# dkogan/mrcal

Measured on AMD Instinct MI355X. Metric: LM (dog-leg) iterations/sec, 8-cam x 1000-frame OPENCV8 calibration, higher is better.
Workload: dtype f64; 1 GPU; 8 cameras x 1000 frames x 10x10 corners, LENSMODEL_OPENCV8, all variables optimized, warp + regularization; Nstate=6140, Nmeasurements=1600080, Nnz_J=37200080, parallelism=single GPU

## Files before the change

mrcal_amd/csrc/assembly.hip:

```cpp
#include "solver_device.hpp"
#include "assembly_splined.hpp"
#include "solver_kernel_decls.hpp"

namespace mrcal_amd {




__device__ __forceinline__
void assemble_frame_block(const DeviceProblem& P, const NormalDims& nd, const OpDev& O, const AssemblyPlan& plan,
                          const double* __restrict__ gram, int f, int o0, int o1 ,
                          int mode, bool do_factor, double lambda,
                          const FactorBuffers& F, double* __restrict__ lds_f)
{
    double* __restrict__ Btf  = lds_f;
    double* __restrict__ Df   = lds_f + 6*nd.Nc;
    double* __restrict__ gf   = Df + 36;
    double* __restrict__ Ls   = gf + 6;
    double* __restrict__ rinv = Ls + 36;
    const int t = threadIdx.x;
#ifdef ASM_TS
    long long ats[16]; int nats = 0;
#define ATS() do { if(t == 0 && nats < 16) ats[nats++] = clock64(); } while(0)
#else
#define ATS()
#endif
    ATS();
    const int e0 = 6*f;
    double* __restrict__ Bt = O.Bt;
    double* __restrict__ D  = O.D;
    double* __restrict__ g  = O.g;

    if(mode == 1)
    {
        for(int i = t; i < 6*nd.Nc + 42; i += blockDim.x) lds_f[i] = 0.0;
        __syncthreads();
        const int npos = gram_stride(P.Ndist);
        for(int ob = o0; ob < o1; ob += 8)
        {
            int col_i[8], col_e[8];
            int obs[8];
#pragma unroll
            for(int u = 0; u < 8; u++)
            {
                const int i = (ob + u < o1) ? ob + u : o0;
                obs[u] = plan.frame_obs ? plan.frame_obs[i] : i;
            }
#pragma unroll
            for(int u = 0; u < 8; u++) { col_i[u] = plan.obs_cols[2*obs[u]]; col_e[u] = plan.obs_cols[2*obs[u]+1]; }
            for(int base = 0; base < npos; base += 2*blockDim.x)
            {
                const int pos0 = base + t;
                double vv[2][8];
                int    rec[2];
#pragma unroll
                for(int w = 0; w < 2; w++)
                {
                    const int pos = pos0 + w*blockDim.x;
                    const int pc  = (pos < npos) ? pos : t;
                    rec[w] = (pos < npos) ? plan.frame_pos[pc] : FRAMEPOS_NONE;
#pragma unroll
                    for(int u = 0; u < 8; u++) vv[w][u] = 0.0;
                    if((rec[w] & 7) != FRAMEPOS_NONE)
                    {
#pragma unroll
                        for(int u = 0; u < 8; u++) vv[w][u] = gram[(size_t)obs[u]*npos + pc];
                    }
                }
#pragma unroll
                for(int w = 0; w < 2; w++)
                {
                    const int kind = rec[w] & 7, a = (rec[w] >> 3) & 7, k = rec[w] >> 6;
                    if(kind == FRAMEPOS_NONE) continue;
                    if(kind == FRAMEPOS_BT_INTRINSICS || kind == FRAMEPOS_BT_EXTRINSICS)
                    {
                        double* __restrict__ row = Btf + a*nd.Nc + k;
#pragma unroll
                        for(int u = 0; u < 8; u++)
                        {
                            const int c = (kind == FRAMEPOS_BT_INTRINSICS) ? col_i[u] : col_e[u];
                            if(ob + u < o1 && c >= 0) row[c] += vv[w][u];
                        }
                    }
                    else
                    {
                        double* __restrict__ dst = (kind == FRAMEPOS_GF)      ? gf + a :
                                                   (kind == FRAMEPOS_BT_WARP) ? Btf + a*nd.Nc + k : Df + a*6 + k;
                        double acc = *dst;
#pragma unroll
                        for(int u = 0; u < 8; u++) if(ob + u < o1) acc += vv[w][u];
                        *dst = acc;
                        if(kind == FRAMEPOS_D_MIRROR) Df[k*6 + a] = acc;
                    }
                }
                ATS();
            }
        }
        __syncthreads();
        ATS();
        for(int i = t; i < 6*nd.Nc; i += blockDim.x) Bt[(size_t)e0*nd.Nc + i] = Btf[i];
        if(t < 36)      D[(size_t)f*36 + t]     = Df[t];
        else if(t < 42) g[nd.E_state0 + e0 + (t-36)] = gf[t-36];
    }
    else
    {
        for(int i = t; i < 6*nd.Nc; i += blockDim.x) Btf[i] = Bt[(size_t)e0*nd.Nc + i];
        if(t < 36)      Df[t]    = D[(size_t)f*36 + t];
        else if(t < 42) gf[t-36] = g[nd.E_state0 + e0 + (t-36)];
        __syncthreads();
    }
    if(!do_factor) return;

    if(t == 0)
    {
        double M[6][6];
#pragma unroll
        for(int i=0;i<6;i++)
#pragma unroll
            for(int j=0;j<6;j++) M[i][j] = Df[i*6+j] + ((i == j) ? lambda : 0.0);
        bool ok = true;
#pragma unroll
        for(int j=0;j<6;j++)
        {
            double d = M[j][j];
#pragma unroll
            for(int k=0;k<j;k++) d -= M[j][k]*M[j][k];
            if(!(d > 0.0)) { ok = false; d = 1.0; }
            d = sqrt(d);
            const double rd = 1.0/d;
            M[j][j] = d;
            rinv[j] = rd;
#pragma unroll
            for(int i=j+1;i<6;i++)
            {
                double v = M[i][j];
#pragma unroll
                for(int k=0;k<j;k++) v -= M[i][k]*M[j][k];
                M[i][j] = v*rd;
            }
        }
#pragma unroll
        for(int i=0;i<6;i++)
#pragma unroll
            for(int j=0;j<6;j++) Ls[i*6+j] = (j <= i) ? M[i][j] : 0.0;
        if(!ok) atomicExch(F.status, 1);
    }
    ATS();
    __syncthreads();
    ATS();
    if(t < 36) F.LD[(size_t)f*36 + t] = Ls[t];
    double Lr[6][6], ri[6];
#pragma unroll
    for(int i=0;i<6;i++)
    {
        ri[i] = rinv[i];
#pragma unroll
        for(int k=0;k<i;k++) Lr[i][k] = Ls[i*6+k];
    }
    for(int c = t; c <= nd.Nc; c += blockDim.x)
    {
        double w[6];
#pragma unroll
        for(int i=0;i<6;i++)
        {
            double v = (c < nd.Nc) ? Btf[i*nd.Nc + c] : gf[i];
#pragma unroll
            for(int k=0;k<i;k++) v -= Lr[i][k]*w[k];
            w[i] = v*ri[i];
        }
        if(c < nd.Nc) { for(int i=0;i<6;i++) F.Wt[(size_t)(e0+i)*nd.Nc + c] = w[i]; }
        else          { for(int i=0;i<6;i++) F.y[e0+i] = w[i]; }
    }
    ATS();
#ifdef ASM_TS
    if(t == 0 && (f == 0 || f == 300 || f == 999))
        printf("asm ts f=%d n=%d (zero | loads + adds | sync | bt-write+factor | sync | fsub): %lld %lld %lld %lld %lld %lld\n", f, nats,
               ats[1]-ats[0], ats[2]-ats[1], ats[3]-ats[2], ats[4]-ats[3], ats[5]-ats[4], ats[6]-ats[5]);
#endif
}

__device__ __forceinline__
void reduce_pair_chunk(const DeviceProblem& P, const AssemblyPlan& plan,
                       const double* __restrict__ gram, int ichunk, int islice )
{
    const int c0 = plan.chunk_begin[ichunk], c1 = plan.chunk_begin[ichunk+1];
    const int npos = gram_stride(P.Ndist);
    const PairOp* __restrict__ ops = plan.pair_table + (size_t)plan.chunk_pair[ichunk]*npos;
    double* __restrict__ out = plan.chunk_part + (size_t)ichunk*npos;
    const int nobs = c1 - c0;
#ifdef ASM_TS
    const long long cts0 = clock64();
#endif
    const int  pos  = islice*blockDim.x + threadIdx.x;
    const int  kind = (pos < npos) ? (ops[pos].op & 0xff) : PAIROP_NONE;
    const bool live = (kind == PAIROP_A || kind == PAIROP_G || kind == PAIROP_NORM);
    double acc = 0.0;
    for(int u0 = 0; u0 < nobs; u0 += 16)
    {
        double vv[16];
        unsigned ob[16];
#pragma unroll
        for(int u = 0; u < 16; u++)
        {
            const int k = (u0 + u < nobs) ? c0 + u0 + u : c0;
            ob[u] = (unsigned)plan.pair_obs[k]*(unsigned)npos;
        }
#pragma unroll
        for(int u = 0; u < 16; u++) vv[u] = 0.0;
        if(live)
        {
// ... 772 lines not shown
```

mrcal_amd/csrc/cholesky_lds.hip:

```cpp
#include "solver_device.hpp"
#include "chol_diag16.hpp"
#include "solver_kernel_decls.hpp"
#include "step_device.hpp"

namespace mrcal_amd {


template<int FINISH>
__device__ __forceinline__
void schur_cholesky_solve_body(int n, const int* __restrict__ skip, int keep_factor,
                               double* __restrict__ S, double* __restrict__ r,
                               int* __restrict__ status, const Step2Dev& sd, const double* __restrict__ Spk = NULL)
{
    if(skip != NULL && *skip) return;
    if constexpr(FINISH == 1) { if(!step2_finish(sd, status)) return; }
    extern __shared__ __attribute__((aligned(16))) double Mp[];
    const int t    = threadIdx.x;
    const int nt   = blockDim.x;
    const int lane = t & 63, wave = t >> 6;
    const int wave_u = __builtin_amdgcn_readfirstlane(wave);
    const int npanels = (n + CHOL_PB - 1)/CHOL_PB;
    const int r16 = lane & 15, kq = lane >> 4;

    auto rowptr = [&](int i) -> double* { return Mp + ((i*(i+1)) >> 1); };
    double* __restrict__ Xs   = Mp + chol_tri_doubles(n);
    double* __restrict__ cbuf = Xs + npanels*CHOL_PB*CHOL_XLD;

    __shared__ int notpd;
    if(t == 0) notpd = 0;
#ifdef CHOL_TS
    long long cts[64]; int ncts = 0;
#define CTS() do { if(t == 0 && ncts < 64) cts[ncts++] = clock64(); } while(0)
#else
#define CTS()
#endif
    CTS();

    if(Spk != NULL)
    {
        const int ntri = ((n*(n + 1)) >> 1) + n;
        const int n16 = min(n, CHOL_PB), nfirst = (n16*(n16 + 1)) >> 1;
        if(wave_u == 0)
        {
            double v[3];
#pragma unroll
            for(int u = 0; u < 3; u++) { const int idx = lane + 64*u; v[u] = Spk[idx < nfirst ? idx : 0]; }
#pragma unroll
            for(int u = 0; u < 3; u++) { const int idx = lane + 64*u; if(idx < nfirst) Mp[idx] = v[u]; }
        }
        else
        {
            constexpr int UP = 16;
            const int nt1 = nt - 64;
            for(int i0 = nfirst + (t - 64); i0 < ntri; i0 += UP*nt1)
            {
                double v[UP];
#pragma unroll
                for(int u = 0; u < UP; u++) { const int idx = i0 + u*nt1; v[u] = Spk[idx < ntri ? idx : 0]; }
#pragma unroll
                for(int u = 0; u < UP; u++) { const int idx = i0 + u*nt1; if(idx < ntri) Mp[idx] = v[u]; }
            }
        }
    }
    else
    {
        double v[13][4];
#pragma unroll
        for(int a = 0; a < 13; a++)
#pragma unroll
            for(int b = 0; b < 4; b++)
                if(b <= a/4)
                {
                    const int  i = wave_u + 16*a, j = lane + 64*b;
                    const bool ok = (i < n && j <= i);
                    v[a][b] = S[ok ? (size_t)i*n + j : 0];
                }
#pragma unroll
        for(int a = 0; a < 13; a++)
#pragma unroll
            for(int b = 0; b < 4; b++)
                if(b <= a/4)
                {
                    const int i = wave_u + 16*a, j = lane + 64*b;
                    if(i < n && j <= i) rowptr(i)[j] = v[a][b];
                }
    }
    if(Spk == NULL)
    {
        for(int j = t; j < n; j += nt) rowptr(n)[j] = r[j];
        __syncthreads();
    }

    auto factor_diag = [&](int p) __attribute__((always_inline))
    {
        const int j0 = p*CHOL_PB;
        const int jb = min(CHOL_PB, n - j0);
        const bool mine = lane < 16 && r16 < jb;
        double* __restrict__ rowL = rowptr(j0 + (mine ? r16 : 0)) + j0;
        double* __restrict__ sink = cbuf + 128 + lane;
        const bool bad = chol_factor_diag16(lane, jb, rowL, Xs + p*CHOL_PB*CHOL_XLD, cbuf,
                                            [&](int c) -> double* { return (mine && c <= r16) ? rowL + c : sink; });
        if(bad && lane == 0) notpd = 1;
    };

    CTS();
    for(int p = -1; p < npanels; p++)
    {
        const int j0 = (p < 0) ? 0 : p*CHOL_PB;
        const int jb = min(CHOL_PB, n - j0);
        const int m0 = j0 + jb;

        if(p >= 0)
        {
            const double* __restrict__ X = Xs + p*CHOL_PB*CHOL_XLD;
            const int ntile_b = (n + 1 - m0 + 15) >> 4;
            for(int ti = wave_u; ti < ntile_b; ti += 16)
            {
                const int  ia = m0 + 16*ti + r16;
                const bool va = ia <= n;
                const double* __restrict__ pa = rowptr(va ? ia : n) + j0;
                chol_double4_t acc = {0.0, 0.0, 0.0, 0.0};
#pragma unroll
                for(int s4 = 0; s4 < 4; s4++)
                {
                    const int  k  = 4*s4 + kq;
                    const bool vk = k < jb;
                    const double al = pa[vk ? k : 0];
                    const double av = (va && vk) ? al : 0.0;
                    const double bv = X[k*CHOL_XLD + r16];
                    acc = __builtin_amdgcn_mfma_f64_16x16x4f64(av, bv, acc, 0, 0, 0);
                }
#pragma unroll
                for(int v = 0; v < 4; v++)
                {
                    const int ri = m0 + 16*ti + kq + 4*v;
                    if(ri <= n && r16 < jb) rowptr(ri)[j0 + r16] = acc[v];
                }
            }
        }
        if(p >= 0) __syncthreads();
        CTS();

        {
            const int nrows = n + 1 - m0, ncols = n - m0;
            const int ntr = (p < 0) ? 0 : (nrows + 15) >> 4, ntc = (ncols + 15) >> 4;
            int ntiles = 0;
            for(int ta = 0; ta < ntr; ta++) ntiles += min(ta + 1, ntc);
            for(int tix = wave_u; tix < ntiles; tix += (wave_u == 0 ? ntiles : 15))
            {
                int ta = 0, tb = tix;
                for(;;) { const int ntb = min(ta + 1, ntc); if(tb < ntb) break; tb -= ntb; ta++; }
                {
                    const int  ia = 16*ta + r16, ib = 16*tb + r16;
                    const bool va = ia < nrows, vb = ib < ncols;
                    const double* __restrict__ pa = rowptr(m0 + (va ? ia : 0)) + j0;
                    const double* __restrict__ pb = rowptr(m0 + (vb ? ib : 0)) + j0;
                    chol_double4_t acc;
                    double* cp[4]; bool cv[4];
#pragma unroll
                    for(int v = 0; v < 4; v++)
                    {
                        const int ri = 16*ta + kq + 4*v, cj = 16*tb + r16;
                        cv[v] = (ri < nrows) && (cj < ncols) && (cj <= ri);
                        cp[v] = rowptr(m0 + (cv[v] ? ri : 0)) + m0 + (cv[v] ? cj : 0);
                        const double cval = *cp[v];
                        acc[v] = cv[v] ? cval : 0.0;
                    }
#pragma unroll
                    for(int s4 = 0; s4 < 4; s4++)
                    {
                        const int  k  = 4*s4 + kq;
                        const bool vk = k < jb;
                        const double al = pa[k], bl = pb[k];
                        const double av = (va && vk) ? -al : 0.0;
                        const double bv = (vb && vk) ?  bl : 0.0;
                        acc = __builtin_amdgcn_mfma_f64_16x16x4f64(av, bv, acc, 0, 0, 0);
                    }
#pragma unroll
                    for(int v = 0; v < 4; v++) if(cv[v]) *cp[v] = acc[v];
                }
            }
            if(wave == 0 && p + 1 < npanels)
            {
                __builtin_amdgcn_s_setprio(3);
                factor_diag(p + 1);
                __builtin_amdgcn_s_setprio(0);
            }
        }
        __syncthreads();
        CTS();
    }
    if(t == 0 && notpd) atomicExch(status, 1);


    double* __restrict__ z = rowptr(n);
    auto back_diag = [&](int p) __attribute__((always_inline))
    {
        const int j0 = p*CHOL_PB;
        const int jb = min(CHOL_PB, n - j0);
        const double* __restrict__ X = Xs + p*CHOL_PB*CHOL_XLD + ((lane < CHOL_PB) ? lane : 0)*CHOL_XLD;
        double xv[CHOL_PB], wv[CHOL_PB];
#pragma unroll
        for(int k = 0; k < CHOL_PB; k++) { xv[k] = X[k]; wv[k] = z[j0 + ((k < jb) ? k : 0)]; }
        double acc0 = 0.0, acc1 = 0.0;
#pragma unroll
        for(int k = 0; k < CHOL_PB; k += 2)
        {
            acc0 += (k   < jb && k   >= lane) ? xv[k]  *wv[k]   : 0.0;
            acc1 += (k+1 < jb && k+1 >= lane) ? xv[k+1]*wv[k+1] : 0.0;
        }
        if(lane < jb) z[j0 + lane] = acc0 + acc1;
    };
    auto back_update = [&](int i, int j0, int jb) __attribute__((always_inline))
    {
        if(jb == CHOL_PB)
        {
            const double* __restrict__ zp = z + j0;
            double lv[CHOL_PB], zv[CHOL_PB];
#pragma unroll
            for(int c = 0; c < CHOL_PB; c++) { lv[c] = rowptr(j0+c)[i]; zv[c] = zp[c]; }
            double acc0 = 0.0, acc1 = 0.0;
#pragma unroll
            for(int c = 0; c < CHOL_PB; c += 2) { acc0 += lv[c]*zv[c]; acc1 += lv[c+1]*zv[c+1]; }
            z[i] -= acc0 + acc1;
        }
        else
        {
            double acc = 0.0;
            for(int c = 0; c < jb; c++) acc += rowptr(j0+c)[i]*z[j0+c];
            z[i] -= acc;
        }
    };
    CTS();
    if(wave == 0 && npanels > 0) back_diag(npanels-1);
    __syncthreads();
    CTS();
    auto back_chain = [&](int p, double& dcur) __attribute__((always_inline))
    {
        const int j0 = p*CHOL_PB, jm = j0 - CHOL_PB, l16 = (lane < CHOL_PB) ? lane : 0;
        const int i = jm + l16;
        const double* __restrict__ X = Xs + (p - 1)*CHOL_PB*CHOL_XLD + l16*CHOL_XLD;
        double lv[CHOL_PB], xv[CHOL_PB];
#pragma unroll
        for(int c = 0; c < CHOL_PB; c++) { lv[c] = rowptr(j0+c)[i]; xv[c] = X[c]; }
        const double zi = z[i];
        double acc0 = 0.0, acc1 = 0.0;
#pragma unroll
        for(int c = 0; c < CHOL_PB; c += 2) { acc0 += lv[c]*readlane_f64(dcur, c); acc1 += lv[c+1]*readlane_f64(dcur, c+1); }
        const double w = zi - (acc0 + acc1);
        double b0 = 0.0, b1 = 0.0;
#pragma unroll
        for(int k = 0; k < CHOL_PB; k += 2)
        {
            const double w0 = readlane_f64(w, k), w1 = readlane_f64(w, k+1);
            b0 += (k   >= lane) ? xv[k]  *w0 : 0.0;
            b1 += (k+1 >= lane) ? xv[k+1]*w1 : 0.0;
        }
        dcur = b0 + b1;
        if(lane < CHOL_PB) z[jm + lane] = dcur;
    };
    double dcur = 0.0;
    bool have_dcur = false;
    for(int p = npanels-1; p >= 1; p--)
    {
        const int j0 = p*CHOL_PB;
        const int jb = min(CHOL_PB, n - j0);
        if(wave == 0)
        {
            if(have_dcur && jb == CHOL_PB) back_chain(p, dcur);
            else
            {
                if(lane < CHOL_PB) back_update(j0 - CHOL_PB + lane, j0, jb);
                back_diag(p - 1);
                dcur = z[j0 - CHOL_PB + ((lane < CHOL_PB) ? lane : 0)];
                have_dcur = true;
            }
        }
        else
            for(int i = t - 64; i < j0 - CHOL_PB; i += nt - 64) back_update(i, j0, jb);
        __syncthreads();
        CTS();
    }
    for(int i = t; i < n; i += nt) r[i] = -z[i];
    if(keep_factor)
        for(int idx = t; idx < n*n; idx += nt)
        {
            const int i = idx / n, j = idx - i*n;
            if(j <= i) S[(size_t)i*n + j] = rowptr(i)[j];
        }
    CTS();
    if constexpr(FINISH != 0) { if(t == 0) step2_chol_done(sd, notpd != 0); }
#ifdef CHOL_TS
    if(t == 0) { printf("chol ts (load | diag0 | b,c per panel ... | backward | store):"); for(int i=1;i<ncts;i++) printf(" %lld", cts[i]-cts[i-1]); printf("\n"); }
#endif
}

template<int FINISH>
__global__ __launch_bounds__(1024)
void schur_cholesky_solve_kernel(int n, const int* __restrict__ skip, int keep_factor,
                                 double* __restrict__ S, double* __restrict__ r,
                                 int* __restrict__ status, Step2Dev sd)
{
    schur_cholesky_solve_body<FINISH>(n, skip, keep_factor, S, r, status, sd);
}

__global__ __launch_bounds__(1024)
void step2_chol_quadform_kernel(int n, int* __restrict__ status, Step2Dev sd, NormalDims nd,
                                double* __restrict__ S, double* __restrict__ r, double* __restrict__ qf_part, int nqf,
                                const double* __restrict__ Spk)
{
    if(blockIdx.x == 0)
    {
// ... 106 lines not shown
```

mrcal_amd/csrc/problem.cpp:

```cpp
#include <hip/hip_runtime.h>
#include <stdlib.h>
#include <string.h>
#include <vector>
#include <map>
#include <algorithm>
#include "layout.hpp"
#include "host_state.hpp"
#include "problem.hpp"
#include "kernels.hpp"
#include "lens_dispatch.hpp"
#include "problem_object.hpp"
#include "host_copy.hpp"
#include <thread>
#include <unordered_map>
#include <mutex>
#include <condition_variable>
#include <deque>
#include <chrono>
#include <unistd.h>

using namespace mrcal_amd;

mrcal_amd_problem::~mrcal_amd_problem()
{
// ... 397 lines not shown
                default: break;
                }
            };
            bool consistent = true;
            for(size_t ip = 0; ip < pair_rep.size(); ip++)
                for(int pos = 0; pos < npos; pos++)
                {
                    int kind, a, k, base;
                    classify(ptab[ip*npos + pos], &kind, &a, &k, &base);
                    if(kind == FRAMEPOS_NONE) continue;
                    const int code = kind | (a << 3) | (k << 6);
                    if(fpos[pos] == FRAMEPOS_NONE) fpos[pos] = code;
                    else if(fpos[pos] != code) consistent = false;
                    if(kind == FRAMEPOS_BT_INTRINSICS || kind == FRAMEPOS_BT_EXTRINSICS)
                    {
                        int& c = pair_cols[2*ip + (kind == FRAMEPOS_BT_EXTRINSICS ? 1 : 0)];
                        if(c < 0) c = base; else if(c != base) consistent = false;
                    }
                }
            for(size_t ip = 0; ip < pair_rep.size() && consistent; ip++)
                for(int pos = 0; pos < npos; pos++)
                {
                    if(eblock_of(meta[pair_rep[ip]]) < 0) break;
                    int kind, a, k, base;
                    classify(ptab[ip*npos + pos], &kind, &a, &k, &base);
                    const int fk = fpos[pos] & 7;
                    const bool absent = (fk == FRAMEPOS_BT_INTRINSICS && pair_cols[2*ip] < 0) || (fk == FRAMEPOS_BT_EXTRINSICS && pair_cols[2*ip+1] < 0);
                    if(kind == FRAMEPOS_NONE ? !(fk == FRAMEPOS_NONE || absent) : absent) consistent = false;
                }
            const bool uses_grams = P->D.lens_type != MRCAL_LENSMODEL_SPLINED_STEREOGRAPHIC;
            if(!consistent && uses_grams) { set_error("internal: the Gram positions of the frame part depend on the camera pair"); return false; }
            std::vector<int> obs_cols(2*(Nobs > 0 ? Nobs : 1), -1);
            for(int o = 0; o < Nobs; o++) { obs_cols[2*o] = pair_cols[2*obs_pair[o]]; obs_cols[2*o+1] = pair_cols[2*obs_pair[o]+1]; }
            ok = ok && P->mem.upload(&P->plan.frame_pos, fpos.data(),     fpos.size());
            ok = ok && P->mem.upload(&P->plan.obs_cols,  obs_cols.data(), obs_cols.size());
        }
        ok = ok && P->mem.upload(&P->plan.obs_pair,   obs_pair.data(),   obs_pair.size());
        ok = ok && P->mem.upload(&P->plan.chunk_pair, chunk_pair.data(), chunk_pair.size());

        const bool with_grams = (L.lensmodel.type != MRCAL_LENSMODEL_SPLINED_STEREOGRAPHIC);
        const int Npairs = with_grams ? (int)pair_rep.size() : 0;
        if(with_grams && npos > 1024)
        {
            set_error("internal error: %d Gram positions per observation", npos);
            return false;
        }
        std::vector<int> pair_chunk_begin(Npairs + 1, 0);
        for(int c=0;c<P->plan.Nchunks && Npairs > 0;c++) pair_chunk_begin[chunk_pair[c] + 1]++;
        for(int ip=0;ip<Npairs;ip++) pair_chunk_begin[ip+1] += pair_chunk_begin[ip];
        const int nA = nd.Nc*nd.Nc, Ndest_all = nA + nd.Nc + 1;
        std::vector<std::vector<int>> src(Npairs > 0 ? Ndest_all : 0);
        for(int ip = 0; ip < Npairs; ip++)
            for(int pos = 0; pos < npos; pos++)
            {
                const PairOp op = ptab[(size_t)ip*npos + pos];
                const int k = op.op & 0xff, code = (ip << 10) | pos;
                if(k == PAIROP_NORM) src[nA + nd.Nc].push_back(code);
                else if(k == PAIROP_G)
                {
                    const int sc = state_to_SE(nd, op.aux);
                    if(sc >= 0) src[nA + sc].push_back(code);
                }
                else if(k == PAIROP_A)
                {
                    const int a = op.aux & 0xffff, b = op.aux >> 16;
                    src[a*nd.Nc + b].push_back(code);
                    if(op.op & PAIROP_MIRROR) src[b*nd.Nc + a].push_back(code);
// ... 973 lines not shown
```

mrcal_amd/csrc/solver_kernels.hpp:

```cpp
#pragma once
#include <hip/hip_runtime.h>
#include <stdint.h>
#include "problem.hpp"
#include "kernels.hpp"

namespace mrcal_amd {

struct NormalDims
{
    int Nstate;
    int Nwarp;
    int i_state_warp;
    int Nc;
    int NE;
    int Nfb;
    int Npb;
    int NEb;
    int S_split, S_shift, E_state0;
    int elim_extrinsics;
};
__host__ __device__ inline int S_to_state(const NormalDims& nd, int s) { return (s < nd.S_split) ? s : s + nd.S_shift; }
__host__ __device__ inline int E_to_state(const NormalDims& nd, int e) { return nd.E_state0 + e; }
__host__ __device__ inline void normal_dims_set_partition(NormalDims& nd, int Nshared_leading)
{
// ... 125 lines not shown
    int     Ndest;
    int*    dest_id; int* dest_begin; int* dest_src; int* group_chunk_begin;
    int     Neblocks;
    int*    eb_block;
    int*    eb_begin;
    int*    eb_rows;
    int*    eb_group;
    int*    eb_epos;
};
struct ReproStep
{
    double*             lvl[3];
    unsigned long long* cmax;
    int*                any;
    size_t              one;
};
bool splined_needs_repro_rows(const DeviceProblem& P);
struct AssemblyPlan
{
    GenPlan gen;
    ReproStep repro;
    int  spl_compact;
    const int* nd_lim;
    int* frame_obs_begin;
    int* frame_obs;
    int* chunk_begin;
    int* pair_obs;
    int* chunk_pair;
    int* obs_pair;
    int  Nchunks, Npairs;
    int*    pos_table;
    PairOp* pair_table;
    int*    frame_pos;
    int*    obs_cols;
    double* chunk_part;
    int*    dest_id;
    int*    dest_begin;
    int*    dest_src;
    int*    pair_chunk_begin;
    int     Ndest;
    double* row_part;
    int     row_part_n;
    double* qf_part;
    int     qf_part_n;
    double* dots_part;
    SplHdr* spl_hdr;
    SplHdr* spl_hdr_extra;
    double* chunk_extra;
    double* spl_part;
};

__host__ __device__ inline int state_to_SE(const NormalDims& nd, int col)
{
    if(col >= nd.E_state0 && col < nd.E_state0 + nd.NE) return -(1 + (col - nd.E_state0));
    return (col < nd.S_split) ? col : col - nd.S_shift;
}
enum { COL_ABSENT = 0, COL_S, COL_FRAME, COL_X };
struct TileColInfo { int kind; int idx; };
__host__ __device__ inline
TileColInfo board_tile_col_info(const DeviceProblem& P, const BoardObsMeta& m, int col)
{
    TileColInfo r = { COL_ABSENT, 0 };
    const int nd = P.Ndist;
    if(col < 4)
    {
        if(P.Ncore_state) { r.kind = COL_S; r.idx = m.i_state_intrinsics + col; }
// ... 131 lines not shown
```

mrcal_amd/csrc/chol_diag16.hpp:

```cpp
#pragma once
#include "solver_device.hpp"

namespace mrcal_amd {

#define CHOL_PB 16
template<int N>
__device__ __forceinline__ double row_share_f64(double v)
{
    union { double d; int i[2]; } u; u.d = v;
    u.i[0] = __builtin_amdgcn_update_dpp(0, u.i[0], 0x150 + N, 0xf, 0xf, true);
    u.i[1] = __builtin_amdgcn_update_dpp(0, u.i[1], 0x150 + N, 0xf, 0xf, true);
    return u.d;
}
typedef double chol_double4_t __attribute__((ext_vector_type(4)));


#define CHOL_XLD 17
__host__ __device__ inline int    chol_tri_doubles(int n) { return ((((n+1)*(n+2)) >> 1) + 1) & ~1; }
__host__ __device__ inline size_t chol_lds_bytes(int n)
{
    const int npanels = (n + CHOL_PB - 1)/CHOL_PB;
    return ((size_t)chol_tri_doubles(n) + (size_t)npanels*CHOL_PB*CHOL_XLD + 3*64)*sizeof(double);
}
static inline bool chol_fits_lds(int n) { return n <= 200 && chol_lds_bytes(n) <= 160*1024 - 4096; }

template<class DstL>
__device__ __forceinline__
bool chol_factor_diag16(const int lane, const int jb, const double* __restrict__ rowL,
                        double* __restrict__ X, double* __restrict__ cbuf, DstL dstL)
{
    const int  r16  = lane & 15;
    const bool mine = lane < 16 && r16 < jb;
#ifdef DIAG16_TS
    const long long dts_in = clock64();
#endif
    double row[CHOL_PB];
    {
        double tmp[CHOL_PB];
#pragma unroll
        for(int c = 0; c < CHOL_PB; c++) tmp[c] = rowL[c];
#pragma unroll
        for(int c = 0; c < CHOL_PB; c++)
            row[c] = mine ? ((c <= r16) ? tmp[c] : 0.0) : ((lane < 32 && c == r16) ? 1.0 : 0.0);
    }
    bool   bad = false;
    double lp[2] = {0.0, 0.0};
    double Lc[2][CHOL_PB];
#pragma unroll
    for(int c = 0; c < CHOL_PB; c++) Lc[0][c] = Lc[1][c] = 0.0;
    double* __restrict__ mycb = cbuf + lane;
#define IC(v) std::integral_constant<int,(v)>{}
    auto column = [&](auto J)
    {
        constexpr int j = decltype(J)::value;
        const double piv = readlane_f64(row[j], j);
// ... 64 lines not shown
```

Measured before the change: 8173 iterations/s.

## Split frame assembly into live-position lists, wave-parallel factor, and prefetch back-substitution loads

```diff
diff --git a/mrcal_amd/csrc/assembly.hip b/mrcal_amd/csrc/assembly.hip
--- a/mrcal_amd/csrc/assembly.hip
+++ b/mrcal_amd/csrc/assembly.hip
@@ -6,6 +6,43 @@
 
 
 
+
+
+__device__ __forceinline__
+bool frame_factor_wave(const double* __restrict__ Df, double lambda, int lane,
+                       double* __restrict__ Ls, double* __restrict__ rinv)
+{
+    const int r = (lane < 6) ? lane : 0;
+    double M[6];
+#pragma unroll
+    for(int j=0;j<6;j++) { const double v = Df[r*6+j]; M[j] = v + ((r == j) ? lambda : 0.0); }
+    bool ok = true;
+#pragma unroll
+    for(int j=0;j<6;j++)
+    {
+        double Mj[6];
+#pragma unroll
+        for(int k=0;k<=j;k++) Mj[k] = readlane_f64(M[k], j);
+        double d = Mj[j];
+#pragma unroll
+        for(int k=0;k<j;k++) d -= Mj[k]*Mj[k];
+        if(!(d > 0.0)) { ok = false; d = 1.0; }
+        d = sqrt(d);
+        const double rd = 1.0/d;
+        if(lane == 0) rinv[j] = rd;
+        double v = M[j];
+#pragma unroll
+        for(int k=0;k<j;k++) v -= M[k]*Mj[k];
+        v = v*rd;
+        M[j] = (lane == j) ? d : v;
+    }
+    if(lane < 6)
+    {
+#pragma unroll
+        for(int j=0;j<6;j++) Ls[lane*6+j] = (j <= lane) ? M[j] : 0.0;
+    }
+    return ok;
+}
 
 __device__ __forceinline__
 void assemble_frame_block(const DeviceProblem& P, const NormalDims& nd, const OpDev& O, const AssemblyPlan& plan,
@@ -19,6 +56,8 @@
     double* __restrict__ Ls   = gf + 6;
     double* __restrict__ rinv = Ls + 36;
     const int t = threadIdx.x;
+    const int lane = t & 63;
+    const int wave = __builtin_amdgcn_readfirstlane(t >> 6);
 #ifdef ASM_TS
     long long ats[16]; int nats = 0;
 #define ATS() do { if(t == 0 && nats < 16) ats[nats++] = clock64(); } while(0)
@@ -35,147 +74,131 @@
     {
         for(int i = t; i < 6*nd.Nc + 42; i += blockDim.x) lds_f[i] = 0.0;
         __syncthreads();
+        ATS();
         const int npos = gram_stride(P.Ndist);
-        for(int ob = o0; ob < o1; ob += 8)
-        {
-            int col_i[8], col_e[8];
-            int obs[8];
-#pragma unroll
-            for(int u = 0; u < 8; u++)
+        const int ndg = plan.frame_ndg, nlive = plan.frame_nlive;
+        const int q0 = (wave == 0) ? lane : ndg + (t - 64), q1 = (wave == 0) ? ndg : nlive;
+        const int qstep = (wave == 0) ? 64 : (int)blockDim.x - 64;
+        for(int q = q0; q < q1; q += qstep)
+        {
+            const int pos = plan.frame_live[q];
+            const int rec = plan.frame_pos[pos];
+            const int kind = rec & 7, a = (rec >> 3) & 7, k = rec >> 6;
+            const bool percam = (kind == FRAMEPOS_BT_INTRINSICS || kind == FRAMEPOS_BT_EXTRINSICS);
+            double* __restrict__ dst = (kind == FRAMEPOS_GF) ? gf + a :
+                                       (kind == FRAMEPOS_D || kind == FRAMEPOS_D_MIRROR) ? Df + a*6 + k : Btf + a*nd.Nc + k;
+            double acc = 0.0;
+            for(int ob = o0; ob < o1; ob += 8)
             {
-                const int i = (ob + u < o1) ? ob + u : o0;
-                obs[u] = plan.frame_obs ? plan.frame_obs[i] : i;
+                int col[8], obs[8];
+                double vv[8];
+#pragma unroll
+                for(int u = 0; u < 8; u++)
+                {
+                    const int i = (ob + u < o1) ? ob + u : o0;
+                    obs[u] = plan.frame_obs ? plan.frame_obs[i] : i;
+                }
+#pragma unroll
+                for(int u = 0; u < 8; u++) col[u] = plan.obs_cols[2*obs[u] + (kind == FRAMEPOS_BT_EXTRINSICS ? 1 : 0)];
+#pragma unroll
+                for(int u = 0; u < 8; u++) vv[u] = gram[(size_t)obs[u]*npos + pos];
+                if(percam)
+                {
+#pragma unroll
+                    for(int u = 0; u < 8; u++)
+                        if(ob + u < o1 && col[u] >= 0) dst[col[u]] += vv[u];
+                }
+                else
+                {
+#pragma unroll
+                    for(int u = 0; u < 8; u++) if(ob + u < o1) acc += vv[u];
+                }
             }
-#pragma unroll
-            for(int u = 0; u < 8; u++) { col_i[u] = plan.obs_cols[2*obs[u]]; col_e[u] = plan.obs_cols[2*obs[u]+1]; }
-            for(int base = 0; base < npos; base += 2*blockDim.x)
+            if(!percam)
             {
-                const int pos0 = base + t;
-                double vv[2][8];
-                int    rec[2];
-#pragma unroll
-                for(int w = 0; w < 2; w++)
-                {
-                    const int pos = pos0 + w*blockDim.x;
-                    const int pc  = (pos < npos) ? pos : t;
-                    rec[w] = (pos < npos) ? plan.frame_pos[pc] : FRAMEPOS_NONE;
-#pragma unroll
-                    for(int u = 0; u < 8; u++) vv[w][u] = 0.0;
-                    if((rec[w] & 7) != FRAMEPOS_NONE)
-                    {
-#pragma unroll
-                        for(int u = 0; u < 8; u++) vv[w][u] = gram[(size_t)obs[u]*npos + pc];
-                    }
-                }
-#pragma unroll
-                for(int w = 0; w < 2; w++)
-                {
-                    const int kind = rec[w] & 7, a = (rec[w] >> 3) & 7, k = rec[w] >> 6;
-                    if(kind == FRAMEPOS_NONE) continue;
-                    if(kind == FRAMEPOS_BT_INTRINSICS || kind == FRAMEPOS_BT_EXTRINSICS)
-                    {
-                        double* __restrict__ row = Btf + a*nd.Nc + k;
-#pragma unroll
-                        for(int u = 0; u < 8; u++)
-                        {
-                            const int c = (kind == FRAMEPOS_BT_INTRINSICS) ? col_i[u] : col_e[u];
-                            if(ob + u < o1 && c >= 0) row[c] += vv[w][u];
-                        }
-                    }
-                    else
-                    {
-                        double* __restrict__ dst = (kind == FRAMEPOS_GF)      ? gf + a :
-                                                   (kind == FRAMEPOS_BT_WARP) ? Btf + a*nd.Nc + k : Df + a*6 + k;
-                        double acc = *dst;
-#pragma unroll
-                        for(int u = 0; u < 8; u++) if(ob + u < o1) acc += vv[w][u];
-                        *dst = acc;
-                        if(kind == FRAMEPOS_D_MIRROR) Df[k*6 + a] = acc;
-                    }
-                }
-                ATS();
+                *dst = acc;
+                if(kind == FRAMEPOS_D_MIRROR) Df[k*6 + a] = acc;
             }
         }
-        __syncthreads();
-        ATS();
-        for(int i = t; i < 6*nd.Nc; i += blockDim.x) Bt[(size_t)e0*nd.Nc + i] = Btf[i];
-        if(t < 36)      D[(size_t)f*36 + t]     = Df[t];
-        else if(t < 42) g[nd.E_state0 + e0 + (t-36)] = gf[t-36];
     }
     else
     {
         for(int i = t; i < 6*nd.Nc; i += blockDim.x) Btf[i] = Bt[(size_t)e0*nd.Nc + i];
         if(t < 36)      Df[t]    = D[(size_t)f*36 + t];
         else if(t < 42) gf[t-36] = g[nd.E_state0 + e0 + (t-36)];
-        __syncthreads();
-    }
-    if(!do_factor) return;
-
-    if(t == 0)
-    {
-        double M[6][6];
+        ATS();
+    }
+    ATS();
+
+    double Lr[6][6], ri[6];
+    auto load_factor = [&]() __attribute__((always_inline))
+    {
 #pragma unroll
         for(int i=0;i<6;i++)
-#pragma unroll
-            for(int j=0;j<6;j++) M[i][j] = Df[i*6+j] + ((i == j) ? lambda : 0.0);
-        bool ok = true;
-#pragma unroll
-        for(int j=0;j<6;j++)
-        {
-            double d = M[j][j];
-#pragma unroll
-            for(int k=0;k<j;k++) d -= M[j][k]*M[j][k];
-            if(!(d > 0.0)) { ok = false; d = 1.0; }
-            d = sqrt(d);
-            const double rd = 1.0/d;
-            M[j][j] = d;
-            rinv[j] = rd;
-#pragma unroll
-            for(int i=j+1;i<6;i++)
+        {
+            ri[i] = rinv[i];
+#pragma unroll
+            for(int k=0;k<i;k++) Lr[i][k] = Ls[i*6+k];
+        }
+    };
+    auto fsub = [&](const double (&bv)[6], double (&w)[6]) __attribute__((always_inline))
+    {
+#pragma unroll
+        for(int i=0;i<6;i++)
+        {
+            double v = bv[i];
+#pragma unroll
+            for(int k=0;k<i;k++) v -= Lr[i][k]*w[k];
+            w[i] = v*ri[i];
+        }
+    };
+    if(wave == 0)
+    {
+        __builtin_amdgcn_fence(__ATOMIC_ACQ_REL, "wavefront");
+        if(mode == 1)
+        {
+            if(t < 36)      D[(size_t)f*36 + t]     = Df[t];
+            else if(t < 42) g[nd.E_state0 + e0 + (t-36)] = gf[t-36];
+        }
+        if(do_factor)
+        {
+            const bool ok = frame_factor_wave(Df, lambda, lane, Ls, rinv);
+            if(!ok && lane == 0) atomicExch(F.status, 1);
+            __builtin_amdgcn_fence(__ATOMIC_ACQ_REL, "wavefront");
+            if(t < 36) F.LD[(size_t)f*36 + t] = Ls[t];
+            load_factor();
+            if(lane == 0)
             {
-                double v = M[i][j];
-#pragma unroll
-                for(int k=0;k<j;k++) v -= M[i][k]*M[j][k];
-                M[i][j] = v*rd;
+                double bv[6], w[6];
+#pragma unroll
+                for(int i=0;i<6;i++) bv[i] = gf[i];
+                fsub(bv, w);
+#pragma unroll
+                for(int i=0;i<6;i++) F.y[e0+i] = w[i];
             }
         }
-#pragma unroll
-        for(int i=0;i<6;i++)
-#pragma unroll
-            for(int j=0;j<6;j++) Ls[i*6+j] = (j <= i) ? M[i][j] : 0.0;
-        if(!ok) atomicExch(F.status, 1);
     }
     ATS();
     __syncthreads();
     ATS();
-    if(t < 36) F.LD[(size_t)f*36 + t] = Ls[t];
-    double Lr[6][6], ri[6];
-#pragma unroll
-    for(int i=0;i<6;i++)
-    {
-        ri[i] = rinv[i];
-#pragma unroll
-        for(int k=0;k<i;k++) Lr[i][k] = Ls[i*6+k];
-    }
-    for(int c = t; c <= nd.Nc; c += blockDim.x)
-    {
-        double w[6];
-#pragma unroll
-        for(int i=0;i<6;i++)
-        {
-            double v = (c < nd.Nc) ? Btf[i*nd.Nc + c] : gf[i];
-#pragma unroll
-            for(int k=0;k<i;k++) v -= Lr[i][k]*w[k];
-            w[i] = v*ri[i];
-        }
-        if(c < nd.Nc) { for(int i=0;i<6;i++) F.Wt[(size_t)(e0+i)*nd.Nc + c] = w[i]; }
-        else          { for(int i=0;i<6;i++) F.y[e0+i] = w[i]; }
+    if(mode == 1)
+        for(int i = t; i < 6*nd.Nc; i += blockDim.x) Bt[(size_t)e0*nd.Nc + i] = Btf[i];
+    if(!do_factor) return;
+    if(wave != 0) load_factor();
+    for(int c = t; c < nd.Nc; c += blockDim.x)
+    {
+        double bv[6], w[6];
+#pragma unroll
+        for(int i=0;i<6;i++) bv[i] = Btf[i*nd.Nc + c];
+        fsub(bv, w);
+#pragma unroll
+        for(int i=0;i<6;i++) F.Wt[(size_t)(e0+i)*nd.Nc + c] = w[i];
     }
     ATS();
 #ifdef ASM_TS
     if(t == 0 && (f == 0 || f == 300 || f == 999))
-        printf("asm ts f=%d n=%d (zero | loads + adds | sync | bt-write+factor | sync | fsub): %lld %lld %lld %lld %lld %lld\n", f, nats,
-               ats[1]-ats[0], ats[2]-ats[1], ats[3]-ats[2], ats[4]-ats[3], ats[5]-ats[4], ats[6]-ats[5]);
+        printf("asm ts f=%d n=%d mode=%d (zero | wave 0: D, g sums | its factorization + y | wait for the Bt sums | bt-write + fsub): %lld %lld %lld %lld %lld\n", f, nats, mode,
+               ats[1]-ats[0], ats[2]-ats[1], ats[3]-ats[2], ats[4]-ats[3], ats[5]-ats[4]);
 #endif
 }
 
diff --git a/mrcal_amd/csrc/cholesky_lds.hip b/mrcal_amd/csrc/cholesky_lds.hip
--- a/mrcal_amd/csrc/cholesky_lds.hip
+++ b/mrcal_amd/csrc/cholesky_lds.hip
@@ -235,15 +235,22 @@
     if(wave == 0 && npanels > 0) back_diag(npanels-1);
     __syncthreads();
     CTS();
-    auto back_chain = [&](int p, double& dcur) __attribute__((always_inline))
+    auto chain_request = [&](int p, double (&lv)[CHOL_PB]) __attribute__((always_inline))
+    {
+        const int j0 = p*CHOL_PB, jm = j0 - CHOL_PB, l16 = (lane < CHOL_PB) ? lane : 0;
+        const int i = jm + l16;
+#pragma unroll
+        for(int c = 0; c < CHOL_PB; c++) lv[c] = rowptr(j0+c)[i];
+    };
+    auto back_chain = [&](int p, double& dcur, const double (&lv)[CHOL_PB]) __attribute__((always_inline))
     {
         const int j0 = p*CHOL_PB, jm = j0 - CHOL_PB, l16 = (lane < CHOL_PB) ? lane : 0;
         const int i = jm + l16;
         const double* __restrict__ X = Xs + (p - 1)*CHOL_PB*CHOL_XLD + l16*CHOL_XLD;
-        double lv[CHOL_PB], xv[CHOL_PB];
-#pragma unroll
-        for(int c = 0; c < CHOL_PB; c++) { lv[c] = rowptr(j0+c)[i]; xv[c] = X[c]; }
         const double zi = z[i];
+        double xv[CHOL_PB];
+#pragma unroll
+        for(int c = 0; c < CHOL_PB; c++) xv[c] = X[c];
         double acc0 = 0.0, acc1 = 0.0;
 #pragma unroll
         for(int c = 0; c < CHOL_PB; c += 2) { acc0 += lv[c]*readlane_f64(dcur, c); acc1 += lv[c+1]*readlane_f64(dcur, c+1); }
@@ -259,15 +266,40 @@
         dcur = b0 + b1;
         if(lane < CHOL_PB) z[jm + lane] = dcur;
     };
+    auto update_request = [&](int i, int j0, double (&lv)[CHOL_PB]) __attribute__((always_inline))
+    {
+#pragma unroll
+        for(int c = 0; c < CHOL_PB; c++) lv[c] = rowptr(j0+c)[i];
+    };
+    auto update_full = [&](int i, int j0, const double (&lv)[CHOL_PB]) __attribute__((always_inline))
+    {
+        const double* __restrict__ zp = z + j0;
+        double zv[CHOL_PB];
+#pragma unroll
+        for(int c = 0; c < CHOL_PB; c++) zv[c] = zp[c];
+        double acc0 = 0.0, acc1 = 0.0;
+#pragma unroll
+        for(int c = 0; c < CHOL_PB; c += 2) { acc0 += lv[c]*zv[c]; acc1 += lv[c+1]*zv[c+1]; }
+        z[i] -= acc0 + acc1;
+    };
     double dcur = 0.0;
     bool have_dcur = false;
+    bool ahead = false;
+    double lv[CHOL_PB];
+    const int irow = t - 64, irow0 = 64*(wave_u - 1);
     for(int p = npanels-1; p >= 1; p--)
     {
         const int j0 = p*CHOL_PB;
         const int jb = min(CHOL_PB, n - j0);
-        if(wave == 0)
-        {
-            if(have_dcur && jb == CHOL_PB) back_chain(p, dcur);
+        const int jm = j0 - CHOL_PB;
+        const bool next = p - 1 >= 1;
+        if(wave_u == 0)
+        {
+            if(have_dcur && jb == CHOL_PB)
+            {
+                if(!ahead) chain_request(p, lv);
+                back_chain(p, dcur, lv);
+            }
             else
             {
                 if(lane < CHOL_PB) back_update(j0 - CHOL_PB + lane, j0, jb);
@@ -275,9 +307,24 @@
                 dcur = z[j0 - CHOL_PB + ((lane < CHOL_PB) ? lane : 0)];
                 have_dcur = true;
             }
+            ahead = next;
+            if(next) chain_request(p - 1, lv);
         }
         else
-            for(int i = t - 64; i < j0 - CHOL_PB; i += nt - 64) back_update(i, j0, jb);
+        {
+            if(jb == CHOL_PB)
+            {
+                if(irow0 < jm)
+                {
+                    if(!ahead) update_request((irow < jm) ? irow : 0, j0, lv);
+                    if(irow < jm) update_full(irow, j0, lv);
+                }
+            }
+            else
+                for(int i = irow; i < jm; i += nt - 64) back_update(i, j0, jb);
+            ahead = next && irow0 < jm - CHOL_PB;
+            if(ahead) update_request((irow < jm - CHOL_PB) ? irow : 0, jm, lv);
+        }
         __syncthreads();
         CTS();
     }
diff --git a/mrcal_amd/csrc/problem.cpp b/mrcal_amd/csrc/problem.cpp
--- a/mrcal_amd/csrc/problem.cpp
+++ b/mrcal_amd/csrc/problem.cpp
@@ -453,7 +453,21 @@
             if(!consistent && uses_grams) { set_error("internal: the Gram positions of the frame part depend on the camera pair"); return false; }
             std::vector<int> obs_cols(2*(Nobs > 0 ? Nobs : 1), -1);
             for(int o = 0; o < Nobs; o++) { obs_cols[2*o] = pair_cols[2*obs_pair[o]]; obs_cols[2*o+1] = pair_cols[2*obs_pair[o]+1]; }
+            std::vector<int> flive;
+            for(int pass = 0; pass < 2; pass++)
+            {
+                for(int pos = 0; pos < npos; pos++)
+                {
+                    const int fk = fpos[pos] & 7;
+                    const bool dg = (fk == FRAMEPOS_D || fk == FRAMEPOS_D_MIRROR || fk == FRAMEPOS_GF);
+                    if(fk != FRAMEPOS_NONE && dg == (pass == 0)) flive.push_back(pos);
+                }
+                if(pass == 0) P->plan.frame_ndg = (int)flive.size();
+            }
+            P->plan.frame_nlive = (int)flive.size();
+            if(flive.empty()) flive.push_back(0);
             ok = ok && P->mem.upload(&P->plan.frame_pos, fpos.data(),     fpos.size());
+            ok = ok && P->mem.upload(&P->plan.frame_live, flive.data(),   flive.size());
             ok = ok && P->mem.upload(&P->plan.obs_cols,  obs_cols.data(), obs_cols.size());
         }
         ok = ok && P->mem.upload(&P->plan.obs_pair,   obs_pair.data(),   obs_pair.size());
diff --git a/mrcal_amd/csrc/solver_kernels.hpp b/mrcal_amd/csrc/solver_kernels.hpp
--- a/mrcal_amd/csrc/solver_kernels.hpp
+++ b/mrcal_amd/csrc/solver_kernels.hpp
@@ -181,6 +181,8 @@
     int*    pos_table;
     PairOp* pair_table;
     int*    frame_pos;
+    int*    frame_live;
+    int     frame_ndg, frame_nlive;
     int*    obs_cols;
     double* chunk_part;
     int*    dest_id;
```

Result: no change. 8098 iterations/s (-0.9%).

## Pad LDS Cholesky to a multiple of 16 with identity rows, removing bounds masks

Applied to the files above, without the earlier changes.

```diff
diff --git a/mrcal_amd/csrc/chol_diag16.hpp b/mrcal_amd/csrc/chol_diag16.hpp
--- a/mrcal_amd/csrc/chol_diag16.hpp
+++ b/mrcal_amd/csrc/chol_diag16.hpp
@@ -16,11 +16,12 @@
 
 
 #define CHOL_XLD 17
-__host__ __device__ inline int    chol_tri_doubles(int n) { return ((((n+1)*(n+2)) >> 1) + 1) & ~1; }
+__host__ __device__ inline int    chol_padded(int n) { return CHOL_PB*((n + CHOL_PB - 1)/CHOL_PB); }
+__host__ __device__ inline int    chol_tri_doubles(int np) { return ((((np+1)*(np+2)) >> 1) + 1) & ~1; }
 __host__ __device__ inline size_t chol_lds_bytes(int n)
 {
-    const int npanels = (n + CHOL_PB - 1)/CHOL_PB;
-    return ((size_t)chol_tri_doubles(n) + (size_t)npanels*CHOL_PB*CHOL_XLD + 3*64)*sizeof(double);
+    const int np = chol_padded(n);
+    return ((size_t)chol_tri_doubles(np) + (size_t)np*CHOL_XLD + 3*64)*sizeof(double);
 }
 static inline bool chol_fits_lds(int n) { return n <= 200 && chol_lds_bytes(n) <= 160*1024 - 4096; }
 
diff --git a/mrcal_amd/csrc/cholesky_lds.hip b/mrcal_amd/csrc/cholesky_lds.hip
--- a/mrcal_amd/csrc/cholesky_lds.hip
+++ b/mrcal_amd/csrc/cholesky_lds.hip
@@ -20,10 +20,11 @@
     const int lane = t & 63, wave = t >> 6;
     const int wave_u = __builtin_amdgcn_readfirstlane(wave);
     const int npanels = (n + CHOL_PB - 1)/CHOL_PB;
+    const int np = npanels*CHOL_PB;
     const int r16 = lane & 15, kq = lane >> 4;
 
     auto rowptr = [&](int i) -> double* { return Mp + ((i*(i+1)) >> 1); };
-    double* __restrict__ Xs   = Mp + chol_tri_doubles(n);
+    double* __restrict__ Xs   = Mp + chol_tri_doubles(np);
     double* __restrict__ cbuf = Xs + npanels*CHOL_PB*CHOL_XLD;
 
     __shared__ int notpd;
@@ -36,9 +37,22 @@
 #endif
     CTS();
 
+
+    const int ntri_n = (n*(n + 1)) >> 1, ntri_np = (np*(np + 1)) >> 1;
+    auto write_padding = [&](int tid, int nthreads)
+    {
+        const int lg = (npanels == 1) ? 4 : 8;
+        for(int id = tid; id < ((np - n) << lg); id += nthreads)
+        {
+            const int i = n + (id >> lg), j = id & ((1 << lg) - 1);
+            if(j <= i) rowptr(i)[j] = (j == i) ? 1.0 : 0.0;
+        }
+        for(int j = n + tid; j < np; j += nthreads) rowptr(np)[j] = 0.0;
+    };
     if(Spk != NULL)
     {
-        const int ntri = ((n*(n + 1)) >> 1) + n;
+        const int ntri = ntri_n + n;
+        const int rhs_shift = ntri_np - ntri_n;
         const int n16 = min(n, CHOL_PB), nfirst = (n16*(n16 + 1)) >> 1;
         if(wave_u == 0)
         {
@@ -47,18 +61,20 @@
             for(int u = 0; u < 3; u++) { const int idx = lane + 64*u; v[u] = Spk[idx < nfirst ? idx : 0]; }
 #pragma unroll
             for(int u = 0; u < 3; u++) { const int idx = lane + 64*u; if(idx < nfirst) Mp[idx] = v[u]; }
+            if(npanels == 1) write_padding(lane, 64);
         }
         else
         {
             constexpr int UP = 16;
             const int nt1 = nt - 64;
+            if(npanels > 1) write_padding(t - 64, nt1);
             for(int i0 = nfirst + (t - 64); i0 < ntri; i0 += UP*nt1)
             {
                 double v[UP];
 #pragma unroll
                 for(int u = 0; u < UP; u++) { const int idx = i0 + u*nt1; v[u] = Spk[idx < ntri ? idx : 0]; }
 #pragma unroll
-                for(int u = 0; u < UP; u++) { const int idx = i0 + u*nt1; if(idx < ntri) Mp[idx] = v[u]; }
+                for(int u = 0; u < UP; u++) { const int idx = i0 + u*nt1; if(idx < ntri) Mp[idx + (idx >= ntri_n ? rhs_shift : 0)] = v[u]; }
             }
         }
     }
@@ -87,18 +103,18 @@
     }
     if(Spk == NULL)
     {
-        for(int j = t; j < n; j += nt) rowptr(n)[j] = r[j];
+        write_padding(t, nt);
+        for(int j = t; j < n; j += nt) rowptr(np)[j] = r[j];
         __syncthreads();
     }
 
     auto factor_diag = [&](int p) __attribute__((always_inline))
     {
         const int j0 = p*CHOL_PB;
-        const int jb = min(CHOL_PB, n - j0);
-        const bool mine = lane < 16 && r16 < jb;
+        const bool mine = lane < 16;
         double* __restrict__ rowL = rowptr(j0 + (mine ? r16 : 0)) + j0;
         double* __restrict__ sink = cbuf + 128 + lane;
-        const bool bad = chol_factor_diag16(lane, jb, rowL, Xs + p*CHOL_PB*CHOL_XLD, cbuf,
+        const bool bad = chol_factor_diag16(lane, CHOL_PB, rowL, Xs + p*CHOL_PB*CHOL_XLD, cbuf,
                                             [&](int c) -> double* { return (mine && c <= r16) ? rowL + c : sink; });
         if(bad && lane == 0) notpd = 1;
     };
@@ -107,26 +123,24 @@
     for(int p = -1; p < npanels; p++)
     {
         const int j0 = (p < 0) ? 0 : p*CHOL_PB;
-        const int jb = min(CHOL_PB, n - j0);
-        const int m0 = j0 + jb;
+        const int m0 = j0 + CHOL_PB;
 
         if(p >= 0)
         {
             const double* __restrict__ X = Xs + p*CHOL_PB*CHOL_XLD;
-            const int ntile_b = (n + 1 - m0 + 15) >> 4;
+            const int ntile_b = (np + 1 - m0 + 15) >> 4;
             for(int ti = wave_u; ti < ntile_b; ti += 16)
             {
                 const int  ia = m0 + 16*ti + r16;
-                const bool va = ia <= n;
-                const double* __restrict__ pa = rowptr(va ? ia : n) + j0;
+                const bool va = ia <= np;
+                const double* __restrict__ pa = rowptr(va ? ia : np) + j0;
                 chol_double4_t acc = {0.0, 0.0, 0.0, 0.0};
 #pragma unroll
                 for(int s4 = 0; s4 < 4; s4++)
                 {
                     const int  k  = 4*s4 + kq;
-                    const bool vk = k < jb;
-                    const double al = pa[vk ? k : 0];
-                    const double av = (va && vk) ? al : 0.0;
+                    const double al = pa[k];
+                    const double av = va ? al : 0.0;
                     const double bv = X[k*CHOL_XLD + r16];
                     acc = __builtin_amdgcn_mfma_f64_16x16x4f64(av, bv, acc, 0, 0, 0);
                 }
@@ -134,7 +148,7 @@
                 for(int v = 0; v < 4; v++)
                 {
                     const int ri = m0 + 16*ti + kq + 4*v;
-                    if(ri <= n && r16 < jb) rowptr(ri)[j0 + r16] = acc[v];
+                    if(ri <= np) rowptr(ri)[j0 + r16] = acc[v];
                 }
             }
         }
@@ -142,26 +156,37 @@
         CTS();
 
         {
-            const int nrows = n + 1 - m0, ncols = n - m0;
-            const int ntr = (p < 0) ? 0 : (nrows + 15) >> 4, ntc = (ncols + 15) >> 4;
-            int ntiles = 0;
-            for(int ta = 0; ta < ntr; ta++) ntiles += min(ta + 1, ntc);
+            const int ncols = np - m0;
+            if(p >= 0 && t >= 64 && t - 64 < ncols)
+            {
+                const int c = t - 64;
+                const double* __restrict__ lr = rowptr(m0 + c) + j0;
+                const double* __restrict__ zr = rowptr(np) + j0;
+                double lv[CHOL_PB], zv[CHOL_PB];
+#pragma unroll
+                for(int k = 0; k < CHOL_PB; k++) { lv[k] = lr[k]; zv[k] = zr[k]; }
+                double acc = rowptr(np)[m0 + c];
+#pragma unroll
+                for(int k = 0; k < CHOL_PB; k++) acc = fma(-zv[k], lv[k], acc);
+                rowptr(np)[m0 + c] = acc;
+            }
+            const int ntc = (p < 0) ? 0 : ncols >> 4;
+            const int ntiles = (ntc*(ntc + 1)) >> 1;
             for(int tix = wave_u; tix < ntiles; tix += (wave_u == 0 ? ntiles : 15))
             {
                 int ta = 0, tb = tix;
-                for(;;) { const int ntb = min(ta + 1, ntc); if(tb < ntb) break; tb -= ntb; ta++; }
+                while(tb > ta) { tb -= ta + 1; ta++; }
                 {
                     const int  ia = 16*ta + r16, ib = 16*tb + r16;
-                    const bool va = ia < nrows, vb = ib < ncols;
-                    const double* __restrict__ pa = rowptr(m0 + (va ? ia : 0)) + j0;
-                    const double* __restrict__ pb = rowptr(m0 + (vb ? ib : 0)) + j0;
+                    const double* __restrict__ pa = rowptr(m0 + ia) + j0;
+                    const double* __restrict__ pb = rowptr(m0 + ib) + j0;
                     chol_double4_t acc;
                     double* cp[4]; bool cv[4];
 #pragma unroll
                     for(int v = 0; v < 4; v++)
                     {
                         const int ri = 16*ta + kq + 4*v, cj = 16*tb + r16;
-                        cv[v] = (ri < nrows) && (cj < ncols) && (cj <= ri);
+                        cv[v] = cj <= ri;
                         cp[v] = rowptr(m0 + (cv[v] ? ri : 0)) + m0 + (cv[v] ? cj : 0);
                         const double cval = *cp[v];
                         acc[v] = cv[v] ? cval : 0.0;
@@ -170,11 +195,8 @@
                     for(int s4 = 0; s4 < 4; s4++)
                     {
                         const int  k  = 4*s4 + kq;
-                        const bool vk = k < jb;
                         const double al = pa[k], bl = pb[k];
-                        const double av = (va && vk) ? -al : 0.0;
-                        const double bv = (vb && vk) ?  bl : 0.0;
-                        acc = __builtin_amdgcn_mfma_f64_16x16x4f64(av, bv, acc, 0, 0, 0);
+                        acc = __builtin_amdgcn_mfma_f64_16x16x4f64(-al, bl, acc, 0, 0, 0);
                     }
 #pragma unroll
                     for(int v = 0; v < 4; v++) if(cv[v]) *cp[v] = acc[v];
@@ -193,46 +215,39 @@
     if(t == 0 && notpd) atomicExch(status, 1);
 
 
-    double* __restrict__ z = rowptr(n);
+    double* __restrict__ z = rowptr(np);
     auto back_diag = [&](int p) __attribute__((always_inline))
     {
         const int j0 = p*CHOL_PB;
-        const int jb = min(CHOL_PB, n - j0);
         const double* __restrict__ X = Xs + p*CHOL_PB*CHOL_XLD + ((lane < CHOL_PB) ? lane : 0)*CHOL_XLD;
         double xv[CHOL_PB], wv[CHOL_PB];
 #pragma unroll
-        for(int k = 0; k < CHOL_PB; k++) { xv[k] = X[k]; wv[k] = z[j0 + ((k < jb) ? k : 0)]; }
+        for(int k = 0; k < CHOL_PB; k++) { xv[k] = X[k]; wv[k] = z[j0 + k]; }
         double acc0 = 0.0, acc1 = 0.0;
 #pragma unroll
         for(int k = 0; k < CHOL_PB; k += 2)
         {
-            acc0 += (k   < jb && k   >= lane) ? xv[k]  *wv[k]   : 0.0;
-            acc1 += (k+1 < jb && k+1 >= lane) ? xv[k+1]*wv[k+1] : 0.0;
-        }
-        if(lane < jb) z[j0 + lane] = acc0 + acc1;
+            acc0 += (k   >= lane) ? xv[k]  *wv[k]   : 0.0;
+            acc1 += (k+1 >= lane) ? xv[k+1]*wv[k+1] : 0.0;
+        }
+        const double d = acc0 + acc1;
+        if(lane < CHOL_PB) z[j0 + lane] = d;
+        return d;
     };
-    auto back_update = [&](int i, int j0, int jb) __attribute__((always_inline))
-    {
-        if(jb == CHOL_PB)
-        {
-            const double* __restrict__ zp = z + j0;
-            double lv[CHOL_PB], zv[CHOL_PB];
-#pragma unroll
-            for(int c = 0; c < CHOL_PB; c++) { lv[c] = rowptr(j0+c)[i]; zv[c] = zp[c]; }
-            double acc0 = 0.0, acc1 = 0.0;
-#pragma unroll
-            for(int c = 0; c < CHOL_PB; c += 2) { acc0 += lv[c]*zv[c]; acc1 += lv[c+1]*zv[c+1]; }
-            z[i] -= acc0 + acc1;
-        }
-        else
-        {
-            double acc = 0.0;
-            for(int c = 0; c < jb; c++) acc += rowptr(j0+c)[i]*z[j0+c];
-            z[i] -= acc;
-        }
+    auto back_update = [&](int i, int j0) __attribute__((always_inline))
+    {
+        const double* __restrict__ zp = z + j0;
+        double lv[CHOL_PB], zv[CHOL_PB];
+#pragma unroll
+        for(int c = 0; c < CHOL_PB; c++) { lv[c] = rowptr(j0+c)[i]; zv[c] = zp[c]; }
+        double acc0 = 0.0, acc1 = 0.0;
+#pragma unroll
+        for(int c = 0; c < CHOL_PB; c += 2) { acc0 += lv[c]*zv[c]; acc1 += lv[c+1]*zv[c+1]; }
+        z[i] -= acc0 + acc1;
     };
     CTS();
-    if(wave == 0 && npanels > 0) back_diag(npanels-1);
+    double dcur = 0.0;
+    if(wave == 0 && npanels > 0) dcur = back_diag(npanels-1);
     __syncthreads();
     CTS();
     auto back_chain = [&](int p, double& dcur) __attribute__((always_inline))
@@ -259,25 +274,12 @@
         dcur = b0 + b1;
         if(lane < CHOL_PB) z[jm + lane] = dcur;
     };
-    double dcur = 0.0;
-    bool have_dcur = false;
     for(int p = npanels-1; p >= 1; p--)
     {
         const int j0 = p*CHOL_PB;
-        const int jb = min(CHOL_PB, n - j0);
-        if(wave == 0)
-        {
-            if(have_dcur && jb == CHOL_PB) back_chain(p, dcur);
-            else
-            {
-                if(lane < CHOL_PB) back_update(j0 - CHOL_PB + lane, j0, jb);
-                back_diag(p - 1);
-                dcur = z[j0 - CHOL_PB + ((lane < CHOL_PB) ? lane : 0)];
-                have_dcur = true;
-            }
-        }
+        if(wave == 0) back_chain(p, dcur);
         else
-            for(int i = t - 64; i < j0 - CHOL_PB; i += nt - 64) back_update(i, j0, jb);
+            for(int i = t - 64; i < j0 - CHOL_PB; i += nt - 64) back_update(i, j0);
         __syncthreads();
         CTS();
     }
```

Result: no change. 7939 iterations/s before, 7898 iterations/s after (-0.5%).
